# HJReachability/ilqgames

Measured on AMD Instinct MI355X. Metric: iLQ iterations/sec (batch), higher is better.
Workload: dtype f64

## Files before the change

### ilqgames_amd/abi.py

```python
import ctypes as C

MAX_PLAYERS = 8
MAX_XDIM = 32

F32, F64 = 0, 1

OK, ERR_INVALID, ERR_UNSUPPORTED, ERR_HIP, ERR_NO_DEVICE = 0, 1, 2, 3, 4

ABI_VERSION = 9
DYN_UNICYCLE_4D, DYN_CAR_5D, DYN_CAR_6D = 1, 2, 3
DYN_UNICYCLE_4D_DISTURBED, DYN_PLANAR_DISTURBANCE = 4, 5
DYN_DUBINS_CAR = 6
DYN_AIR_3D_EVADER, DYN_AIR_3D_PURSUER = 7, 8
DYN_POINT_MASS_2D = 9
DYN_UNICYCLE_5D = 10
DYN_CAR_7D = 11
DYN_DELAYED_DUBINS_CAR = 12
(COST_QUADRATIC, COST_QUADRATIC_POLYLINE2, COST_SEMIQUADRATIC, COST_SEMIQUADRATIC_POLYLINE2,
 COST_PROXIMITY, COST_SIGNED_DISTANCE, COST_EXTREME_VALUE, CONSTRAINT_PROXIMITY,
 CONSTRAINT_SINGLE_DIMENSION) = range(1, 10)
COST_POLYLINE2_SIGNED_DISTANCE = 10
COST_QUADRATIC_DIFFERENCE = 11
COST_ORIENTATION = 12
COST_QUADRATIC_NORM = 13
# ... 28 lines not shown
CHOICE_AUTO, CHOICE_OFF, CHOICE_ON = 0, 1, 2
SWEEP_GENERIC = 3


class InstanceParam(C.Structure):
    _fields_ = [("term", C.c_int32), ("field", C.c_int32)]


PARAM_WEIGHT, PARAM_VALUE = 0, 1
PARAM_FIELDS = {"weight": PARAM_WEIGHT, "value": PARAM_VALUE}


class IterateLog(C.Structure):
    _fields_ = [("xs", C.c_void_p), ("us", C.c_void_p), ("costs", C.c_void_p), ("P", C.c_void_p),
                ("alpha", C.c_void_p), ("count", C.c_void_p), ("capacity", C.c_int32)]


class SolveOptions(C.Structure):
    _fields_ = [("fixed_iters", C.c_int32), ("augmented_lagrangian", C.c_int32), ("resume", C.c_int32),
                ("deterministic", C.c_int32), ("active", C.c_void_p), ("forced_steps", C.c_void_p),
                ("split_trial", C.c_int32), ("handoff", C.c_int32), ("probe", C.c_int32), ("counted", C.c_int32),
                ("compact_rows", C.c_int32), ("round_bursts", C.c_int32), ("generic_kernels", C.c_int32),
                ("probe_first", C.c_int32), ("single_wave_sweep", C.c_int32), ("adjoint_expected_decrease", C.c_int32),
                ("static_rows", C.c_int32), ("padded_sweep", C.c_int32), ("probe_lanes", C.c_int32), ("reserved2", C.c_int32),
                ("iterate_log", C.POINTER(IterateLog)), ("max_runtime", C.c_double)]


class Subsystem(C.Structure):
    _fields_ = [("kind", C.c_int32), ("xdim", C.c_int32), ("udim", C.c_int32), ("param0", C.c_float)]


class CostTerm(C.Structure):
    _fields_ = [("kind", C.c_int32), ("role", C.c_int32), ("player", C.c_int32), ("arg", C.c_int32),
                ("idx", C.c_int32 * 4), ("idx_extra", C.c_int32 * 2), ("weight", C.c_float), ("value", C.c_float),
                ("value2", C.c_float),
                ("flags", C.c_int32),
                ("polyline", C.c_int32), ("child_begin", C.c_int32), ("child_count", C.c_int32),
                ("constraint_slot", C.c_int32), ("first_step", C.c_int32)]


class PlayerCost(C.Structure):
    _fields_ = [("state_regularization", C.c_float), ("control_regularization", C.c_float),
                ("structure", C.c_int32)]


class SolverParams(C.Structure):
    _fields_ = [("convergence_tolerance", C.c_float), ("max_solver_iters", C.c_int32),
# ... 337 lines not shown
```

### ilqgames_amd/csrc/ilqg_api.hip

```cpp
#include <hip/hip_runtime.h>

#include <cstdio>
#include <cstdlib>
#include <cmath>
#include <chrono>
#include <cstring>
#include <string>
#include <vector>

#include "ilqg_common.hpp"
#include "ilqg_lq.hpp"
#include "ilqg_lq_openloop.hpp"
#include "ilqg_lq_feedback2.hpp"
#include "ilqg_lq_generic.hpp"
#include "ilqg_costates.hpp"
#include "ilqg_models.hpp"
#include "ilqg_nash.hpp"
#include "ilqg_receding.hpp"
#include "ilqg_rowprog.hpp"
#include "ilqg_rowprog_static.hpp"
#include "ilqg_solve.hpp"
#include "ilqg_stages.hpp"

using namespace ilqg;
// ... 393 lines not shown
}
template <typename T>
__global__ void __launch_bounds__(64) ilq_deadline_kernel(DevProblem p, SolveArgs<T> sa) {
  deadline_part_instance<T>(p, sa, int(blockIdx.x));
}

template <typename T, int NX, int NP, int MU>
__global__ void __launch_bounds__(256) ilq_exit_kernel(DevProblem p, SolveArgs<T> sa) {
  extern __shared__ __align__(16) unsigned char smem_raw[];
  const int b = blockIdx.x;
  {
    const WsLayout L(p.n, p.m, p.N, p.T, p.pairs.Rsz, p.pairs.rsz, sa.ol_row, p.num_constraints, sa.al_mode);
    const int stage = reinterpret_cast<const SolveState<T>*>(sa.ws + size_t(b) * sa.ws_stride + L.state)->stage;
    if (stage != ST_INNER_DONE) return;
  }
  const QuadTables<T> tb = quad_tables_load<T>(p, smem_raw, b);
  T* sm = reinterpret_cast<T*>(smem_raw + quad_tables_bytes(p, sizeof(T)));
  exit_part_instance<T, NX, NP, MU>(p, tb, sa, b, sm);
}

#ifndef ILQG_1W_WAVES_F64
#define ILQG_1W_WAVES_F64 2
#endif
template <typename T, int NX, int NP, int MU, int KIND>
__global__ void __launch_bounds__((KIND == LQ_SINGLE_WAVE ? 64 : KIND == LQ_VALU_FEEDBACK ? LQCfg<T, NX, NP, MU>::NT : ((KIND == LQ_OPEN_LOOP || KIND == LQ_OPEN_LOOP_COMPACT) ? OLCfg<T, NX, NP, MU>::NT : 64 * NP)),
                                  (KIND == LQ_SINGLE_WAVE ? (sizeof(T) == 4 ? 4 : ILQG_1W_WAVES_F64) : KIND == LQ_PLAYER_WAVES_PACKED ? 4 : KIND == LQ_PLAYER_WAVES ? (NX <= 16 ? NP : 2) : ((KIND == LQ_OPEN_LOOP || KIND == LQ_OPEN_LOOP_COMPACT) ? 3 : 1)))
ilq_lq_kernel(DevProblem p, SolveArgs<T> sa) {
  extern __shared__ __align__(16) unsigned char smem_raw[];
  const int b = blockIdx.x;
  if (sa.clear_counters && b == 0 && threadIdx.x < 4) sa.unfinished[threadIdx.x] = 0;
  {
    const WsLayout L(p.n, p.m, p.N, p.T, p.pairs.Rsz, p.pairs.rsz, sa.ol_row, p.num_constraints, sa.al_mode);
    const int stage = reinterpret_cast<const SolveState<T>*>(sa.ws + size_t(b) * sa.ws_stride + L.state)->stage;
    if (stage != ST_LQ) return;
  }
  lq_part_instance<T, NX, NP, MU, (KIND == LQ_PLAYER_WAVES_PACKED ? LQ_PLAYER_WAVES : KIND)>(p, sa, b, reinterpret_cast<T*>(smem_raw));
}

template <typename T, int NX, int NP, int MU, bool OL>
struct PadLayout {
  static constexpr int M = NP * MU;
  size_t A, B, Q, l, R, r, P, al, dx, scr, x0, total;
  __host__ __device__ PadLayout(int T_steps, int Rsz, int rsz) {
    size_t o = 0;
    auto take = [&](size_t cnt) {
      const size_t at = o;
      o += (cnt + 3) & ~size_t(3);
      return at;
    };
    const size_t Tn = size_t(T_steps);
    A = take(Tn * NX * NX);
    B = take(Tn * NX * M);
    Q = take(Tn * NP * NX * NX);
    l = take(Tn * NP * NX);
    R = take(Tn * Rsz);
    r = take(Tn * rsz);
    P = take(Tn * M * NX);
    al = take(Tn * M);
    dx = take(Tn * NX);
// ... 914 lines not shown
  const bool lists = split || handoff;
  sa.defer_forward = (!split && !open_loop) ? 1 : 0;
  {
    constexpr size_t fwd_elems = 4 * 2 * ((NX * NX + C::SCR + 3) & ~3) + 2 * NX + 8;
    if (trial_rows_elems(d, sa.rows_cw, static_prog != 0) < fwd_elems + 8) sa.defer_forward = 0;
  }
  const bool adjoint = choice(opt.adjoint_expected_decrease, sa.defer_forward == 0);
  const bool single_wave = has_1w && pw && sa.compact && !kProfile && (adjoint || sa.defer_forward) &&
                           d.rp_compact_w <= W1Cfg<T, NX, NP, MU>::kWords &&
                           choice(opt.single_wave_sweep, !opt.deterministic && size_t(sched_batch) >= size_t(5) * num_cus);
  if (single_wave) {
    sa.prio_div = 0;
    if (adjoint) sa.defer_forward = 0;
  }
  constexpr bool has_packed = sizeof(T) == 4 && C::USE_MFMA && C::MFMA_ONE_TILE && NP == 3;
  if (open_loop) {
    plan.sweep = {ol_compact ? ilq_lq_kernel<T, NX, NP, MU, LQ_OPEN_LOOP_COMPACT> : ilq_lq_kernel<T, NX, NP, MU, LQ_OPEN_LOOP>,
                  O::NT, (O::LDS_ELEMS + 4) * sizeof(T)};
  } else if constexpr (!C::USE_MFMA) {
    plan.sweep = {ilq_lq_kernel<T, NX, NP, MU, LQ_VALU_FEEDBACK>, C::NT, C::LDS_ELEMS * sizeof(T)};
  } else {
    plan.sweep = {ilq_lq_kernel<T, NX, NP, MU, LQ_PLAYER_WAVES>, 64 * NP,
                  (MfmaSweepLds<T, NX, NP, MU>::ELEMS + (C::MFMA_ONE_TILE ? 0 : 4)) * sizeof(T)};
    if constexpr (has_packed)
      if (size_t(sched_batch) >= size_t(5) * 256) plan.sweep.kernel = ilq_lq_kernel<T, NX, NP, MU, LQ_PLAYER_WAVES_PACKED>;
    if constexpr (has_1w)
      if (single_wave) plan.sweep = {ilq_lq_kernel<T, NX, NP, MU, LQ_SINGLE_WAVE>, 64, size_t(W1Cfg<T, NX, NP, MU>::ELEMS + 4) * sizeof(T)};
  }
  sa.clear_counters = 1;
  plan.trial = {k_trial, 64 * W, lds_trial};
  plan.exit = {ilq_exit_kernel<T, NX, NP, MU>, nt_exit, quad_tables_bytes(d, sizeof(T)) + 64 * sizeof(T)};
  plan.read_restarts = counted && al_mode;
  constexpr bool pairs = rollout_pairs(NX, NP, MU);
  if (lists) {
    const size_t lds_roll = trial_phase_lds_bytes<T>(d, TRIAL_ROLL, sa.rows_cw);
    const size_t lds_proll = pairs ? size_t(rollout_pair_lds_elems(d.n, d.m)) * sizeof(T) + 16 : lds_roll;
    const size_t static_regs_lds = (rows_state_in_registers(NX, NP * MU) ? 0 : size_t(d.n + d.m) * 64) * sizeof(T) + 16;
    const int rows_cw = static_id ? 64 : sa.rows_cw;
    const bool regs = static_id && static_in_regs;
    plan.roll = {ilq_roll_kernel<T, NX, NP, MU>, 64, lds_proll};
    plan.rows = {k_rows, 64, regs ? static_regs_lds : split_maps_bytes + split_rows_elems(d, NX, rows_cw) * sizeof(T)};
    plan.decide = {ilq_decide_kernel<T, NX, NP, MU>, 64, trial_phase_lds_bytes<T>(d, TRIAL_DECIDE, sa.rows_cw)};
    plan.prows = {k_prows, 64, regs ? static_regs_lds : split_maps_bytes + probe_rows_elems(d, NX, rows_cw) * sizeof(T)};
    plan.proll = {ilq_probe_roll_kernel<T, NX, NP, MU>, 64, lds_proll};
    plan.proll_fat = {ilq_probe_roll_kernel<T, NX, NP, MU, sizeof(T) == 8>, 64, lds_proll};
    if (pairs) {
      plan.proll_single = {ilq_probe_roll_kernel<T, NX, NP, MU, sizeof(T) == 8, true>, 64, lds_roll};
      plan.proll_lanes = {ilq_probe_roll_lanes_kernel<T, NX, NP, MU>, 64, size_t(rollout_lanes_lds_elems(d.n, d.m, d.N)) * sizeof(T) + 16};
    }
  }
// ... 509 lines not shown

ilqg_status ilqg_solve_batch_ex(ilqg_problem* p, int32_t batch, const void* x0, void* xs, void* us, void* P,
                                void* alpha, void* total_costs, int32_t* iters, int32_t* status, int32_t* converged,
                                void* workspace, const ilqg_solve_options* options, void* stream) {
  if (!p || !x0 || !xs || !us || !P || !alpha || !total_costs || !iters || !status || !converged || !workspace || !options)
    return fail(ILQG_ERR_INVALID, "null argument");
  if (batch <= 0) return ILQG_OK;
  if (ilqg_status sb = instance_batch_check(p, batch)) return sb;
  const ilqg_solve_options& o = *options;
  if (o.fixed_iters < 0) return fail(ILQG_ERR_INVALID, "fixed_iters must not be negative");
  if (o.forced_steps && (o.fixed_iters <= 0 || o.augmented_lagrangian))
    return fail(ILQG_ERR_INVALID, "forced_steps needs fixed_iters > 0 and no augmented-Lagrangian loop");
  if (o.max_runtime > 0.0 && (o.fixed_iters > 0 || o.forced_steps))
    return fail(ILQG_ERR_INVALID, "max_runtime needs a free-running solve (fixed_iters = 0, no forced steps)");
  if (o.single_wave_sweep < ILQG_CHOICE_AUTO || o.single_wave_sweep > ILQG_CHOICE_ON ||
      o.adjoint_expected_decrease < ILQG_CHOICE_AUTO || o.adjoint_expected_decrease > ILQG_CHOICE_ON)
    return fail(ILQG_ERR_INVALID, "scheduling choices are ilqg_choice values");
  if (o.probe_first < 0 || o.probe_first > 1024) return fail(ILQG_ERR_INVALID, "probe_first: 0 (the library's choice) or a count");
  for (int32_t c : {o.split_trial, o.handoff, o.probe, o.counted})
    if (c < ILQG_CHOICE_AUTO || c > ILQG_CHOICE_ON) return fail(ILQG_ERR_INVALID, "scheduling choices are ilqg_choice values");
  const DevProblem& d = p->dev;
  hipStream_t st = (hipStream_t)stream;
  if (o.generic_kernels < ILQG_CHOICE_AUTO || o.generic_kernels > ILQG_CHOICE_ON || o.padded_sweep < ILQG_CHOICE_AUTO ||
      o.padded_sweep > ILQG_CHOICE_ON || o.probe_lanes < ILQG_CHOICE_AUTO || o.probe_lanes > ILQG_CHOICE_ON)
    return fail(ILQG_ERR_INVALID, "scheduling choices are ilqg_choice values");
  if (p->generic || o.generic_kernels == ILQG_CHOICE_ON)
    return p->desc.dtype == ILQG_F32
               ? generic_solve<float>(p, batch, x0, xs, us, P, alpha, total_costs, iters, status, converged, workspace, o, st)
               : generic_solve<double>(p, batch, x0, xs, us, P, alpha, total_costs, iters, status, converged, workspace, o, st);
#define X(NX_, NP_, MU_)                                                                                        \
  if (d.n == NX_ && d.N == NP_ && p->mu_uniform == MU_) {                                                       \
    return p->desc.dtype == ILQG_F32                                                                            \
               ? DimsLaunch<float, NX_, NP_, MU_>::solve(p, batch, x0, xs, us, P, alpha, total_costs, iters, status,  \
                                                         converged, workspace, o, st)                            \
               : DimsLaunch<double, NX_, NP_, MU_>::solve(p, batch, x0, xs, us, P, alpha, total_costs, iters, status, \
                                                          converged, workspace, o, st);                          \
  }
  ILQG_FOR_DIMS(X)
#undef X
  return fail(ILQG_ERR_UNSUPPORTED, "no device kernel instantiated for this problem's dimensions");
}

ilqg_status ilqg_ilq_solve_batch(ilqg_problem* p, int32_t batch, const void* x0, void* xs, void* us, void* P,
                                 void* alpha, void* total_costs, int32_t* iters, int32_t* status, int32_t* converged,
                                 void* workspace, int32_t fixed_iters, void* stream) {
  ilqg_solve_options o;
  ilqg_default_solve_options(&o);
// ... 281 lines not shown
```

### ilqgames_amd/csrc/ilqg_lq.hpp

```cpp
#pragma once

#include "ilqg_common.hpp"
#include "ilqg_mfma.hpp"

namespace ilqg {

template <typename T>
struct LQArgs {
  const T *A, *Bm, *Q, *l, *R, *r;
  const T* x0;
  T *P, *alpha, *dx;
  T* scratch;
  T* ed_out;
  T* costates = nullptr;
  int T_steps;
  int adaptive;
  int symmetric = 0;
  int defer_forward = 0;
  long long* ph = nullptr;
  const T* compact = nullptr;
  const int* compact_tab = nullptr;
  double dt = 0.0;
  int prio_div = 0;
  long long* tl = nullptr;
// ... 170 lines not shown
template <typename T, int M>
__device__ __forceinline__ void lu_solve_columns(T (&col)[M], int lane, T (&x)[M]) {
  T dinv[M];
#pragma unroll
  for (int k = 0; k + 1 < M; k++) {
    const T rinv = fast_recip(col[k]);
    dinv[k] = bcast(rinv, k);
    T f[M];
#pragma unroll
    for (int i = k + 1; i < M; i++) f[i] = bcast(col[i] * rinv, k);
#pragma unroll
    for (int i = k + 1; i < M; i++) col[i] -= f[i] * col[k];
  }
  dinv[M - 1] = bcast(fast_recip(col[M - 1]), M - 1);
#pragma unroll
  for (int i = M - 1; i >= 0; i--) {
    T s = col[i];
#pragma unroll
    for (int k2 = i + 1; k2 < M; k2++) s -= bcast(col[i], k2) * x[k2];
    x[i] = s * dinv[i];
  }
}

template <typename T, int M>
__device__ __forceinline__ void lu_pp_solve_columns(T (&col)[M], int lane, T (&x)[M]) {
#pragma unroll
  for (int k = 0; k + 1 < M; k++) {
    int p = k;
    T best = col[k] < T(0) ? -col[k] : col[k];
#pragma unroll
    for (int i = k + 1; i < M; i++) {
      const T v = col[i] < T(0) ? -col[i] : col[i];
      const bool gt = v > best;
      best = gt ? v : best;
      p = gt ? i : p;
    }
    p = __builtin_amdgcn_readlane(p, k);
    const T ck = col[k];
    T cp = ck;
#pragma unroll
    for (int i = k + 1; i < M; i++) {
      const bool sel = (i == p);
      cp = sel ? col[i] : cp;
      col[i] = sel ? ck : col[i];
    }
    col[k] = cp;
// ... 516 lines not shown
  static constexpr int PS = ((NX * int(sizeof(T))) % 16 == 0 && (LD * int(sizeof(T))) % 16 == 0) ? 16 : 4;
  static constexpr int WAVE_INSTRS = (16 * LD * int(sizeof(T)) / PS + 63) / 64;
};

template <typename T, int NX, int LD, int PS, int WI>
__device__ __forceinline__ void dma_tile(const T* g_, T* tile, int nrows, int ncols, int lane) {
  const T* g = uniform_ptr(g_);
  constexpr int COLB = LD * int(sizeof(T));
#pragma unroll
  for (int h = 0; h < WI; h++) {
    const int pos = (64 * h + lane) * PS;
    const int c = pos / COLB, inb = pos % COLB;
    if (c < ncols && inb + PS <= nrows * int(sizeof(T))) {
      const char* src = reinterpret_cast<const char*>(g) + unsigned(c * NX * int(sizeof(T)) + inb);
      char* dst = reinterpret_cast<char*>(tile) + 64 * h * PS;
      if constexpr (PS == 16)
        __builtin_amdgcn_global_load_lds((glb_vptr)src, (lds_vptr)dst, 16, 0, 0);
      else
        __builtin_amdgcn_global_load_lds((glb_vptr)src, (lds_vptr)dst, 4, 0, 0);
    }
  }
}

template <typename T, int NX, int NP, int MU, bool SOLVER = false>
__device__ __forceinline__ void lq_feedback_instance_mfma_pw(const LQArgs<T>& a, const PairTable& pt, T* sm) {
  using C = LQCfg<T, NX, NP, MU>;
  using W = PWCfg<T, NX, NP, MU>;
  using TL = Tile<T>;
  using vec = typename TL::vec;
  constexpr int M = C::M, NT = 64 * NP, NS = C::NSOLVE, S = int(sizeof(T)), LD = W::LD;
  static_assert(M <= 16 && NS <= 32, "the Nash system must fit two 16-column tiles");
  constexpr bool SPARE = NX < 16;
  constexpr int JB = SPARE ? NX : 0;
  const int t = threadIdx.x;
  const int w = t >> 6;
  const int lane = t & 63, g = lane >> 4, j = lane & 15;
  const int Tn = a.T_steps;
  const PairRegs<NP> pr(pt);
  const bool want_fwd = SOLVER || a.dx != nullptr || a.ed_out != nullptr || a.defer_forward != 0;
  constexpr int SCR = C::SCR;
  const vec zero4 = {T(0), T(0), T(0), T(0)};
  constexpr int RS = TL::row(0, 1) - TL::row(0, 0);
  const int row0 = TL::row(g, 0);
  const int offD = row0 + LD * j;
  const int offT = j + LD * row0;
  auto ldD = [&](const T* tile) {
    vec v;
// ... 313 lines not shown
    }
    ILQG_PH(1);
    if (cmp) dma_wait();
    lds_sync(false);
    ILQG_PH(7);
    if (NP > 1 && w != 0) {
      if (k > 0) {
        if (cmp)
          stage_c(k - 1, 1 - cur, w - 1, HELPERS);
        else
          stage(k - 1, 1 - cur, w - 1, HELPERS);
      }
      ILQG_PH(14);
      if constexpr (!SOLVER)
      {
        stash_ql(k);
        if (w == 1) stash_ql_of(k, 0);
      }
      ILQG_PH(15);
    }

    if (w == 0) {
      T col[M], x[M];
      const bool isS = lane < M;
      const T* src = (lane < M + NX) ? sSY + M * lane : sYz;
#pragma unroll
      for (int r = 0; r < M; r++) {
        col[r] = src[r];
        x[r] = T(0);
      }
      {
        T l1 = T(0);
#pragma unroll
        for (int r = 0; r < M; r++) l1 += lq_abs(col[r]);
        const T diag = src[isS ? lane : 0];
        const T radius = l1 - lq_abs(diag);
        const T eval_lo = diag - radius;
        const T bump = (isS && adaptive && eval_lo < T(1e-3f)) ? radius + T(1e-3f) : T(0);
#pragma unroll
        for (int r = 0; r < M; r++) col[r] = col[r] + ((r == lane) ? bump : T(0));
      }
      ILQG_PH(10);
      if (adaptive)
        lu_solve_columns<T, M>(col, lane, x);
      else
        qr_solve_columns<T, M>(col, lane, x);
      ILQG_PH(11);
      if constexpr (SPARE) {
        if (lane >= M && lane <= M + NX) {
#pragma unroll
          for (int r = 0; r < M; r++) sPt[r + LD * (lane - M)] = x[r];
        }
      } else {
        if (lane >= M && lane < M + NX) {
#pragma unroll
          for (int r = 0; r < M; r++) sPt[r + LD * (lane - M)] = x[r];
        } else if (lane == M + NX) {
#pragma unroll
          for (int r = 0; r < M; r++) sAl[r] = x[r];
        }
      }
    }
    ILQG_PH(2);
    lds_sync(false);
    ILQG_PH(8);
    if (w == NP - 1) {
      typedef __attribute__((address_space(1))) T gT;
      if (lane < NX) {
        T pv[M];
#pragma unroll
        for (int r = 0; r < M; r++) pv[r] = sPt[r + LD * lane];
        gT* dst = (gT*)(uniform_ptr(a.P + size_t(k) * M * NX)) + unsigned(M * lane);
#pragma unroll
        for (int r = 0; r < M; r++) dst[r] = pv[r];
      } else if (lane < NX + M) {
        ((gT*)(uniform_ptr(a.alpha + size_t(k) * M)))[unsigned(lane - NX)] = sAlr[lane - NX];
      }
    }

    const vec Pd = ldD(sPt);
// ... 299 lines not shown
```

### ilqgames_amd/csrc/ilqg_lq_feedback1w.hpp

```cpp
#pragma once

#include "ilqg_lq.hpp"

namespace ilqg {

template <typename T, int NX, int NP, int MU>
struct W1Cfg {
  using C = LQCfg<T, NX, NP, MU>;
  static constexpr int M = NP * MU;
  static constexpr int LD = sizeof(T) == 8 ? 18 : 17;
  static constexpr int TILE = (16 * LD + 3) & ~3;
  static constexpr int oTA = 0;
  static constexpr int oTB = oTA + TILE;
  static constexpr int oTQ = oTB + TILE;
  static constexpr int oVl = oTQ + NP * TILE;
  static constexpr int oVR = (oVl + NP * NX + 3) & ~3;
  static constexpr int oVr = (oVR + C::RMAX + 3) & ~3;
  static constexpr int IMG = (oVr + C::rMAX + 3) & ~3;
  static constexpr int oPt = IMG;
  static constexpr int oAl = oPt + TILE;
  static constexpr int oYz = oAl + 16;
  static constexpr bool SY_IN_PT = M * 32 <= TILE;
  static constexpr int oSY = SY_IN_PT ? oPt : oYz + 16;
  static constexpr int oG = oYz + 16 + (SY_IN_PT ? 0 : M * 32);
  static constexpr int kWords = 192;
  static constexpr int oSB = oG + NP * MU * 16;
  static constexpr int oCD = oSB + kWords;
  static constexpr int CD_ELEMS = (kWords * 4 + int(sizeof(T)) - 1) / int(sizeof(T));
  static constexpr int oQL = (oCD + CD_ELEMS + 3) & ~3;
  static constexpr int oMu = oQL + NP * 16;
  static constexpr int ELEMS = (oMu + 32 + 3) & ~3;
  static constexpr bool SUPPORTED = NX < 16 && M <= 16 && C::NSOLVE <= 32 && NP <= 4 && MU == 2;
};

template <typename T, int NX, int NP, int MU>
__device__ __forceinline__ void lq_feedback_instance_mfma_1w(const LQArgs<T>& a, const PairTable& pt, T* sm) {
  using C = LQCfg<T, NX, NP, MU>;
  using W = W1Cfg<T, NX, NP, MU>;
  using TL = Tile<T>;
  using vec = typename TL::vec;
  constexpr int M = C::M, S = int(sizeof(T)), LD = W::LD, SCR = C::SCR, JB = NX;
  static_assert(W::SUPPORTED, "the single-wave sweep needs a spare tile column (n < 16) and a Nash system of <= 32 columns");
  const int lane = threadIdx.x & 63, g = lane >> 4, j = lane & 15;
  const int Tn = a.T_steps;
  const PairRegs<NP> pr(pt);
  const vec zero4 = {T(0), T(0), T(0), T(0)};
  constexpr int RS = TL::row(0, 1) - TL::row(0, 0);
  const int row0 = TL::row(g, 0);
  const int offD = row0 + LD * j;
  const int offT = j + LD * row0;
  auto ldD = [&](const T* tile) {
    vec v;
#pragma unroll
    for (int r = 0; r < 4; r++) v[r] = tile[offD + RS * r];
    return v;
  };
  auto ldDT = [&](const T* tile) {
    vec v;
// ... 168 lines not shown
#pragma unroll
        for (int q = 0; q < MU; q++) pS[q] = pY[q] = T(0);
#pragma unroll
        for (int r = 0; r < 4; r++) {
          const T* gp = sGw + (row0 + RS * r) * MU;
#pragma unroll
          for (int q = 0; q < MU; q++) {
            const T gval = gp[q];
            pS[q] += gval * Bd[r];
            pY[q] += gval * Ad[r];
          }
        }
        const T tot = rows_reduce4<T>(pS[0], pS[1], pY[0], pY[1]);
        const bool diag = !isY && j / MU == w;
        const T rd = sR[pr.ro[w][w] + aa + MU * (diag ? j - w * MU : 0)];
        const T val = tot + (diag ? rd : T(0));
        if (isY ? j < NX : j < M) sSY[(w * MU + aa) + M * c] = val;
      }
    }
    lds_sync(true);

    {
      T col[M], x[M];
      const bool isS = lane < M;
      const T* src = (lane < M + NX) ? sSY + M * lane : sYz;
#pragma unroll
      for (int r = 0; r < M; r++) {
        col[r] = src[r];
        x[r] = T(0);
      }
      {
        T l1 = T(0);
#pragma unroll
        for (int r = 0; r < M; r++) l1 += lq_abs(col[r]);
        const T diag = src[isS ? lane : 0];
        const T radius = l1 - lq_abs(diag);
        const T eval_lo = diag - radius;
        const T bump = (isS && a.adaptive && eval_lo < T(1e-3f)) ? radius + T(1e-3f) : T(0);
#pragma unroll
        for (int r = 0; r < M; r++) col[r] = col[r] + ((r == lane) ? bump : T(0));
      }
      if (a.adaptive)
        lu_solve_columns<T, M>(col, lane, x);
      else
        qr_solve_columns<T, M>(col, lane, x);
      if (lane >= M && lane <= M + NX) {
#pragma unroll
        for (int r = 0; r < M; r++) sPt[r + LD * (lane - M)] = x[r];
      }
    }
    lds_sync(true);
    {
      typedef __attribute__((address_space(1))) T gT;
      if (lane < NX) {
        T pv[M];
#pragma unroll
        for (int r = 0; r < M; r++) pv[r] = sPt[r + LD * lane];
        gT* dst = (gT*)(uniform_ptr(a.P + size_t(k) * M * NX)) + unsigned(M * lane);
#pragma unroll
        for (int r = 0; r < M; r++) dst[r] = pv[r];
      } else if (lane < NX + M) {
        ((gT*)(uniform_ptr(a.alpha + size_t(k) * M)))[unsigned(lane - NX)] = sAl[lane - NX];
      }
    }

    const vec Pd = ldD(sPt);
    vec nBT = ldDT(tB);
#pragma unroll
    for (int r = 0; r < 4; r++) nBT[r] = -nBT[r];
    const vec Fd = tile_xty_blocks<T, kblock_mask<T>(0, M)>(nBT, Pd, Ad);
    T muv[4] = {T(0), T(0), T(0), T(0)};
// ... 111 lines not shown
```

### ilqgames_amd/csrc/ilqg_solve.hpp

```cpp
#pragma once
#ifndef ILQG_ROLL_PRIO
#define ILQG_ROLL_PRIO 1
#endif

#include "ilqg_lq.hpp"
#include "ilqg_lq_openloop.hpp"
#include "ilqg_lq_feedback2.hpp"
#include "ilqg_lq_feedback1w.hpp"
#include "ilqg_lq_generic.hpp"
#include "ilqg_stages.hpp"

namespace ilqg {

template <typename T>
struct SolveArgs {
  const T* x0;
  T *xs, *us;
  T *P, *alpha;
  T* total_costs;
  int *iters, *status, *converged;
  const int* active;
  T* ws;
  size_t ws_stride;
  int fixed_iters;
// ... 893 lines not shown
  if (size_t(t) < N) lg.costs[at * N + t] = sa.total_costs[size_t(b) * N + t];
  if (lg.P) {
    const T* P = ib.PB(s.sacc);
    for (size_t e = t; e < Tn * m * n; e += nt) lg.P[at * Tn * m * n + e] = P[e];
  }
  if (lg.alpha) {
    const T* al = ib.AL(s.sacc);
    for (size_t e = t; e < Tn * m; e += nt) lg.alpha[at * Tn * m + e] = al[e] * s.acc_scale;
  }
}

template <typename T>
__device__ __forceinline__ void deadline_part_instance(const DevProblem& p, const SolveArgs<T>& sa, int b) {
  const WsLayout L(p.n, p.m, p.N, p.T, p.pairs.Rsz, p.pairs.rsz, sa.ol_row, p.num_constraints, sa.al_mode);
  SolveState<T>* const st = reinterpret_cast<SolveState<T>*>(sa.ws + size_t(b) * sa.ws_stride + L.state);
  if (threadIdx.x == 0 && st->stage == ST_LQ) {
    st->stage = ST_INNER_DONE;
    atomicAdd(sa.unfinished + 1, 1);
  }
}

enum { LQ_VALU_FEEDBACK = 0, LQ_PLAYER_WAVES = 1, LQ_OPEN_LOOP = 2, LQ_PLAYER_WAVES_PACKED = 3, LQ_OPEN_LOOP_COMPACT = 4,
       LQ_SINGLE_WAVE = 5 };
template <typename T, int NX, int NP, int MU, int KIND>
__device__ __forceinline__ void lq_part_instance(const DevProblem& p, const SolveArgs<T>& sa, int b, T* sm) {
  const int Tn = p.T;
  const WsLayout L(p.n, p.m, p.N, p.T, p.pairs.Rsz, p.pairs.rsz, sa.ol_row, p.num_constraints, sa.al_mode);
  T* const w = sa.ws + size_t(b) * sa.ws_stride;
  SolveState<T>* const st = reinterpret_cast<SolveState<T>*>(w + L.state);
  const int sacc = __builtin_amdgcn_readfirstlane(st->sacc);
  const long long pr_start = clock64();
  LQArgs<T> la;
  la.A = w + L.A;
  la.Bm = w + L.B;
  la.Q = w + L.Q;
  la.l = w + L.l;
  la.R = w + L.R;
  la.r = w + L.r;
  la.x0 = nullptr;
  la.P = sacc ? sa.P + size_t(b) * Tn * p.m * p.n : w + L.P1;
  la.alpha = sacc ? sa.alpha + size_t(b) * Tn * p.m : w + L.al1;
  constexpr bool kOL = KIND == LQ_OPEN_LOOP || KIND == LQ_OPEN_LOOP_COMPACT;
  const bool defer = sa.defer_forward && !kOL;
  la.dx = defer ? nullptr : w + L.dx;
  la.defer_forward = defer ? 1 : 0;
  la.scratch = w + L.lqscr;
  constexpr int ed_slot = kOL ? OLCfg<T, NX, NP, MU>::LDS_ELEMS
// ... 7 lines not shown
  if constexpr (kOL) {
    bool blocks = true;
#pragma unroll
    for (int i = 0; i < NP; i++) blocks = blocks && p.xoff[i + 1] > p.xoff[i];
    if (blocks) {
      la.nsub = NP;
#pragma unroll
      for (int i = 0; i <= NP; i++) la.xoff[i] = p.xoff[i];
    }
  }
  la.prio_div = KIND == LQ_PLAYER_WAVES ? sa.prio_div : 0;
  if (sa.compact && (KIND == LQ_PLAYER_WAVES || KIND == LQ_OPEN_LOOP_COMPACT || KIND == LQ_SINGLE_WAVE)) {
    la.compact = w + L.Q;
    la.compact_tab = p.row_prog + p.rp_compact_off;
    la.dt = p.dt;
  }
  la.ph = (kProfile && sa.prof) ? sa.prof + size_t(b) * 96 + 8 : nullptr;
  la.tl = kTimeline ? sa.prof : nullptr;
  la.tl_b = b;
  tl_stamp(sa.prof, b, 16, threadIdx.x == 0);
  if constexpr (KIND == LQ_PLAYER_WAVES) {
    if constexpr (LQCfg<T, NX, NP, MU>::MFMA_ONE_TILE) {
      if (la.compact != nullptr && defer)
        lq_feedback_instance_mfma_pw<T, NX, NP, MU, true>(la, p.pairs, sm);
      else
        lq_feedback_instance_mfma<T, NX, NP, MU>(la, p.pairs, sm);
    } else
    lq_feedback_instance_mfma<T, NX, NP, MU>(la, p.pairs, sm);
  } else if constexpr (KIND == LQ_SINGLE_WAVE) {
    if constexpr (W1Cfg<T, NX, NP, MU>::SUPPORTED) {
      la.dx = nullptr;
      lq_feedback_instance_mfma_1w<T, NX, NP, MU>(la, p.pairs, sm);
    }
  } else if constexpr (KIND == LQ_OPEN_LOOP) {
    lq_openloop_instance<T, NX, NP, MU>(la, p.pairs, sm);
  } else if constexpr (KIND == LQ_OPEN_LOOP_COMPACT) {
    lq_openloop_instance<T, NX, NP, MU, true>(la, p.pairs, sm);
  } else {
    lq_feedback_instance<T, NX, NP, MU>(la, p.pairs, sm);
  }
  __syncthreads();
  tl_stamp(sa.prof, b, 19, threadIdx.x == 0);
  if (threadIdx.x == 0) {
    if (defer)
      st->ed_pending = 1;
    else
      st->expected_decrease = sm[ed_slot];
    st->num_iterations += 1;
    st->step = sa.forced_steps ? sa.forced_steps[size_t(b) * sa.fixed_iters + (st->num_iterations - 1)]
                               : T(sa.prm.initial_alpha_scaling);
    st->bt = 0;
    st->stage = ST_ROLLOUT;
    if (kProfile && sa.prof) sa.prof[size_t(b) * 96 + 2] += clock64() - pr_start;
  }
}
// ... 43 lines not shown
```

### ilqgames_amd/hip.py

```python
import ctypes as C
import os

import numpy as np

from . import abi

_HERE = os.path.dirname(os.path.abspath(__file__))
LIB_PATH = os.environ.get("ILQG_HIP_LIB") or os.path.join(_HERE, "libilqg_hip.so")
_LIB = None

EXPORTS = [
    "ilqg_lq_feedback_batch", "ilqg_lq_openloop_batch", "ilqg_default_solver_params", "ilqg_problem_create",
    "ilqg_problem_destroy", "ilqg_workspace_bytes", "ilqg_rollout_batch", "ilqg_linearize_batch",
    "ilqg_quadraticize_batch", "ilqg_problem_pairs", "ilqg_total_costs_batch", "ilqg_ilq_solve_batch",
    "ilqg_last_error", "ilqg_abi_version", "ilqg_device_info", "ilqg_selftest_mfma", "ilqg_al_solve_batch", "ilqg_plan_integrate_batch", "ilqg_receding_horizon_sync_batch",
    "ilqg_solution_splice_batch", "ilqg_solve_again_batch", "ilqg_strategy_costs_batch",
    "ilqg_check_local_nash_batch", "ilqg_check_sufficient_nash_batch",
    "ilqg_receding_horizon_shift_batch", "ilqg_default_solve_options", "ilqg_solve_batch_ex", "ilqg_solve_state_batch",
    "ilqg_set_scratch", "ilqg_problem_last_schedule", "ilqg_copy_bandwidth", "ilqg_problem_row_program", "ilqg_row_program_build",
    "ilqg_problem_declare_instance_params", "ilqg_problem_bind_instance_values", "ilqg_instance_params_check",
]


class IlqgError(RuntimeError):
# ... 219 lines not shown
        te = torch.zeros((B, self.N), dtype=torch.int32, device="cuda") if t_extreme is None else \
            torch.as_tensor(np.ascontiguousarray(t_extreme, dtype=np.int32), device="cuda")
        _check(lib().ilqg_total_costs_batch(self.h, B, _ptr(xs), _ptr(us), _ptr(costs), _ptr(te), None, _stream()))
        return costs, te

    def workspace_bytes(self, batch):
        b = C.c_uint64(0)
        _check(lib().ilqg_workspace_bytes(self.h, batch, C.byref(b)))
        return b.value

    def alloc_solve_buffers(self, batch):
        import torch
        z = lambda *s: torch.zeros(s, dtype=torch_dtype(self.dtype), device="cuda")
        return dict(xs=z(batch, self.T, self.n), us=z(batch, self.T, self.m), P=z(batch, self.T, self.m * self.n),
                    alpha=z(batch, self.T, self.m), costs=z(batch, self.N),
                    iters=torch.zeros(batch, dtype=torch.int32, device="cuda"),
                    status=torch.zeros(batch, dtype=torch.int32, device="cuda"),
                    converged=torch.zeros(batch, dtype=torch.int32, device="cuda"),
                    ws=torch.empty(self.workspace_bytes(batch), dtype=torch.uint8, device="cuda"))

    def solve(self, x0, bufs=None, fixed_iters=0, augmented_lagrangian=False, forced_steps=None, split_trial=None,
              handoff=None, probe=None, counted=None, resume=False, active=None, compact_rows=None, round_bursts=None,
              log_capacity=0, log_strategies=False, max_runtime=0.0, generic_kernels=None, probe_first=0, single_wave_sweep=None, adjoint_expected_decrease=None,
              deterministic=False, static_rows=None, padded_sweep=None, probe_lanes=None):
        import torch
        x0 = _dev(x0, self.dtype)
        B = x0.shape[0]
        if bufs is None:
            bufs = self.alloc_solve_buffers(B)
        o = abi.SolveOptions()
        lib().ilqg_default_solve_options(C.byref(o))
        o.fixed_iters = int(fixed_iters)
        o.augmented_lagrangian = 1 if augmented_lagrangian else 0
        o.resume = 1 if resume else 0
        o.deterministic = 1 if deterministic else 0
        o.active = None if active is None else active.data_ptr()
        fs = None
        if forced_steps is not None:
            fs = _dev(forced_steps, self.dtype)
            assert tuple(fs.shape) == (B, fixed_iters)
            o.forced_steps = fs.data_ptr()
        tri = lambda v: abi.CHOICE_AUTO if v is None else (abi.CHOICE_ON if v else abi.CHOICE_OFF)
        o.split_trial, o.handoff, o.probe, o.counted = tri(split_trial), tri(handoff), tri(probe), tri(counted)
        o.compact_rows = tri(compact_rows)
        o.round_bursts = tri(round_bursts)
        o.generic_kernels = tri(generic_kernels)
        o.probe_first = int(probe_first)
        o.single_wave_sweep = tri(self.single_wave_sweep if single_wave_sweep is None else single_wave_sweep)
        o.adjoint_expected_decrease = tri(adjoint_expected_decrease)
        o.static_rows = tri(static_rows)
        o.padded_sweep = tri(padded_sweep)
        o.probe_lanes = tri(probe_lanes)
        o.max_runtime = float(max_runtime)
        il = None
        if log_capacity > 0:
            cap = int(log_capacity)
            log = dict(xs=self._empty(B, cap, self.T, self.n), us=self._empty(B, cap, self.T, self.m),
                       costs=self._empty(B, cap, self.N), count=torch.zeros(B, dtype=torch.int32, device="cuda"))
            if log_strategies:
                log["P"] = self._empty(B, cap, self.T, self.m * self.n)
                log["alpha"] = self._empty(B, cap, self.T, self.m)
            il = abi.IterateLog(log["xs"].data_ptr(), log["us"].data_ptr(), log["costs"].data_ptr(),
                                log["P"].data_ptr() if log_strategies else None,
                                log["alpha"].data_ptr() if log_strategies else None, log["count"].data_ptr(), cap)
            o.iterate_log = C.pointer(il)
            bufs["log"] = log
        _check(lib().ilqg_solve_batch_ex(self.h, B, _ptr(x0), _ptr(bufs["xs"]), _ptr(bufs["us"]), _ptr(bufs["P"]),
                                         _ptr(bufs["alpha"]), _ptr(bufs["costs"]), _ptr(bufs["iters"]),
                                         _ptr(bufs["status"]), _ptr(bufs["converged"]), _ptr(bufs["ws"]), C.byref(o),
                                         _stream()))
        return bufs

    def solve_state(self, bufs, augmented_lagrangian=False):
        import torch
        B = bufs["iters"].shape[0]
# ... 144 lines not shown
```

### include/ilqg.h

```cpp
#ifndef ILQG_H_
#define ILQG_H_

#include <stddef.h>
#include <stdint.h>

#ifdef __cplusplus
extern "C" {
#endif

#define ILQG_MAX_PLAYERS 8
#define ILQG_MAX_XDIM 32
#define ILQG_MAX_UDIM_TOTAL 16
#define ILQG_MAX_PAIRS 64

typedef enum {
  ILQG_OK = 0,
  ILQG_ERR_INVALID = 1,
  ILQG_ERR_UNSUPPORTED = 2,
  ILQG_ERR_HIP = 3,
  ILQG_ERR_NO_DEVICE = 4
} ilqg_status;

typedef enum { ILQG_F32 = 0, ILQG_F64 = 1 } ilqg_dtype;

// ... 206 lines not shown
                                 void* workspace, int32_t fixed_iters,
                                 void* stream);

typedef struct {
  int32_t fixed_iters;
  int32_t augmented_lagrangian;
  int32_t resume;
  int32_t deterministic;
  const int32_t* active;
  const void* forced_steps;
  int32_t split_trial;
  int32_t handoff;
  int32_t probe;
  int32_t counted;
  int32_t compact_rows;
  int32_t round_bursts;
  int32_t generic_kernels;
  int32_t probe_first;
  int32_t single_wave_sweep;
  int32_t adjoint_expected_decrease;
  int32_t static_rows;
  int32_t padded_sweep;
  int32_t probe_lanes;
  int32_t reserved2;
  const struct ilqg_iterate_log* iterate_log;
  double max_runtime;
} ilqg_solve_options;

typedef struct ilqg_iterate_log {
  void* xs;
  void* us;
  void* costs;
  void* P;
  void* alpha;
  int32_t* count;
  int32_t capacity;
} ilqg_iterate_log;
void ilqg_default_solve_options(ilqg_solve_options* o);

ilqg_status ilqg_solve_batch_ex(ilqg_problem* p, int32_t batch, const void* x0, void* xs, void* us, void* P,
                                void* alpha, void* total_costs, int32_t* iters, int32_t* status, int32_t* converged,
                                void* workspace, const ilqg_solve_options* options, void* stream);

ilqg_status ilqg_solve_state_batch(const ilqg_problem* p, int32_t batch, const void* workspace,
                                   int32_t augmented_lagrangian, void* last_merit, void* expected_decrease,
                                   void* step, int32_t* backtracks, void* stream);

// ... 80 lines not shown
```

Before: 1.997 million.

## Solve feedback LU system with row-replicated DPP broadcasts instead of lane-per-column elimination

Adds a row-broadcast LU solve path for the per-step coupled Nash system in the player-wave and single-wave MFMA sweeps. Each 16-lane row holds a replicated copy of the M matrix columns plus a slice of the right-hand sides, and pivot values are shared with DPP row_bcast instead of cross-lane shuffles across the full wave. The goal is to shorten the dependent elimination chain and spread the right-hand sides across rows. It is enabled by default through a new sweep_forms option, with the old kernels kept as fallbacks. This path always uses unpivoted LU, even when the adaptive flag would otherwise select QR, so robustness may change for ill-conditioned systems.

```diff
diff --git a/ilqgames_amd/abi.py b/ilqgames_amd/abi.py
--- a/ilqgames_amd/abi.py
+++ b/ilqgames_amd/abi.py
@@ -74,7 +74,7 @@
                 ("split_trial", C.c_int32), ("handoff", C.c_int32), ("probe", C.c_int32), ("counted", C.c_int32),
                 ("compact_rows", C.c_int32), ("round_bursts", C.c_int32), ("generic_kernels", C.c_int32),
                 ("probe_first", C.c_int32), ("single_wave_sweep", C.c_int32), ("adjoint_expected_decrease", C.c_int32),
-                ("static_rows", C.c_int32), ("padded_sweep", C.c_int32), ("probe_lanes", C.c_int32), ("reserved2", C.c_int32),
+                ("static_rows", C.c_int32), ("padded_sweep", C.c_int32), ("probe_lanes", C.c_int32), ("sweep_forms", C.c_int32),
                 ("iterate_log", C.POINTER(IterateLog)), ("max_runtime", C.c_double)]
 
 
diff --git a/ilqgames_amd/csrc/ilqg_api.hip b/ilqgames_amd/csrc/ilqg_api.hip
--- a/ilqgames_amd/csrc/ilqg_api.hip
+++ b/ilqgames_amd/csrc/ilqg_api.hip
@@ -439,7 +439,7 @@
 #ifndef ILQG_1W_WAVES_F64
 #define ILQG_1W_WAVES_F64 2
 #endif
-template <typename T, int NX, int NP, int MU, int KIND>
+template <typename T, int NX, int NP, int MU, int KIND, bool FORMS = true>
 __global__ void __launch_bounds__((KIND == LQ_SINGLE_WAVE ? 64 : KIND == LQ_VALU_FEEDBACK ? LQCfg<T, NX, NP, MU>::NT : ((KIND == LQ_OPEN_LOOP || KIND == LQ_OPEN_LOOP_COMPACT) ? OLCfg<T, NX, NP, MU>::NT : 64 * NP)),
                                   (KIND == LQ_SINGLE_WAVE ? (sizeof(T) == 4 ? 4 : ILQG_1W_WAVES_F64) : KIND == LQ_PLAYER_WAVES_PACKED ? 4 : KIND == LQ_PLAYER_WAVES ? (NX <= 16 ? NP : 2) : ((KIND == LQ_OPEN_LOOP || KIND == LQ_OPEN_LOOP_COMPACT) ? 3 : 1)))
 ilq_lq_kernel(DevProblem p, SolveArgs<T> sa) {
@@ -451,7 +451,7 @@
     const int stage = reinterpret_cast<const SolveState<T>*>(sa.ws + size_t(b) * sa.ws_stride + L.state)->stage;
     if (stage != ST_LQ) return;
   }
-  lq_part_instance<T, NX, NP, MU, (KIND == LQ_PLAYER_WAVES_PACKED ? LQ_PLAYER_WAVES : KIND)>(p, sa, b, reinterpret_cast<T*>(smem_raw));
+  lq_part_instance<T, NX, NP, MU, (KIND == LQ_PLAYER_WAVES_PACKED ? LQ_PLAYER_WAVES : KIND), FORMS>(p, sa, b, reinterpret_cast<T*>(smem_raw));
 }
 
 template <typename T, int NX, int NP, int MU, bool OL>
@@ -1412,10 +1412,24 @@
   } else {
     plan.sweep = {ilq_lq_kernel<T, NX, NP, MU, LQ_PLAYER_WAVES>, 64 * NP,
                   (MfmaSweepLds<T, NX, NP, MU>::ELEMS + (C::MFMA_ONE_TILE ? 0 : 4)) * sizeof(T)};
-    if constexpr (has_packed)
-      if (size_t(sched_batch) >= size_t(5) * 256) plan.sweep.kernel = ilq_lq_kernel<T, NX, NP, MU, LQ_PLAYER_WAVES_PACKED>;
-    if constexpr (has_1w)
-      if (single_wave) plan.sweep = {ilq_lq_kernel<T, NX, NP, MU, LQ_SINGLE_WAVE>, 64, size_t(W1Cfg<T, NX, NP, MU>::ELEMS + 4) * sizeof(T)};
+    constexpr bool has_forms = C::MFMA_ONE_TILE && SolveRows<NP * MU, NX + 1>::FITS;
+    const bool forms = choice(opt.sweep_forms, true);
+    if constexpr (has_forms)
+      if (!forms) plan.sweep.kernel = ilq_lq_kernel<T, NX, NP, MU, LQ_PLAYER_WAVES, false>;
+    if constexpr (has_packed) {
+      if (size_t(sched_batch) >= size_t(5) * 256) {
+        plan.sweep.kernel = ilq_lq_kernel<T, NX, NP, MU, LQ_PLAYER_WAVES_PACKED>;
+        if constexpr (has_forms)
+          if (!forms) plan.sweep.kernel = ilq_lq_kernel<T, NX, NP, MU, LQ_PLAYER_WAVES_PACKED, false>;
+      }
+    }
+    if constexpr (has_1w) {
+      if (single_wave) {
+        plan.sweep = {ilq_lq_kernel<T, NX, NP, MU, LQ_SINGLE_WAVE>, 64, size_t(W1Cfg<T, NX, NP, MU>::ELEMS + 4) * sizeof(T)};
+        if constexpr (has_forms)
+          if (!forms) plan.sweep.kernel = ilq_lq_kernel<T, NX, NP, MU, LQ_SINGLE_WAVE, false>;
+      }
+    }
   }
   sa.clear_counters = 1;
   plan.trial = {k_trial, 64 * W, lds_trial};
@@ -1971,7 +1985,8 @@
   const DevProblem& d = p->dev;
   hipStream_t st = (hipStream_t)stream;
   if (o.generic_kernels < ILQG_CHOICE_AUTO || o.generic_kernels > ILQG_CHOICE_ON || o.padded_sweep < ILQG_CHOICE_AUTO ||
-      o.padded_sweep > ILQG_CHOICE_ON || o.probe_lanes < ILQG_CHOICE_AUTO || o.probe_lanes > ILQG_CHOICE_ON)
+      o.padded_sweep > ILQG_CHOICE_ON || o.probe_lanes < ILQG_CHOICE_AUTO || o.probe_lanes > ILQG_CHOICE_ON ||
+      o.sweep_forms < ILQG_CHOICE_AUTO || o.sweep_forms > ILQG_CHOICE_ON)
     return fail(ILQG_ERR_INVALID, "scheduling choices are ilqg_choice values");
   if (p->generic || o.generic_kernels == ILQG_CHOICE_ON)
     return p->desc.dtype == ILQG_F32
diff --git a/ilqgames_amd/csrc/ilqg_lq.hpp b/ilqgames_amd/csrc/ilqg_lq.hpp
--- a/ilqgames_amd/csrc/ilqg_lq.hpp
+++ b/ilqgames_amd/csrc/ilqg_lq.hpp
@@ -216,6 +216,44 @@
   }
 }
 
+template <int M, int NRHS>
+struct SolveRows {
+  static constexpr int PER = 16 - M;
+  static constexpr bool FITS = M >= 1 && M < 16 && 4 * PER >= NRHS;
+};
+template <int K>
+__device__ __forceinline__ float row_bcast(float v) {
+  return __builtin_amdgcn_mov_dpp(v, 0x150 + K, 0xf, 0xf, false);
+}
+template <int K>
+__device__ __forceinline__ double row_bcast(double v) {
+  return __builtin_amdgcn_mov_dpp(v, 0x150 + K, 0xf, 0xf, false);
+}
+template <typename T, int M>
+__device__ __forceinline__ void lu_solve_columns_rows(T (&col)[M], T (&x)[M]) {
+  T dinv[M];
+  static_for<M - 1>([&](auto K) {
+    constexpr int k = decltype(K)::value;
+    const T rinv = fast_recip(col[k]);
+    dinv[k] = row_bcast<k>(rinv);
+    T f[M];
+#pragma unroll
+    for (int i = k + 1; i < M; i++) f[i] = row_bcast<k>(col[i] * rinv);
+#pragma unroll
+    for (int i = k + 1; i < M; i++) col[i] -= f[i] * col[k];
+  });
+  dinv[M - 1] = row_bcast<M - 1>(fast_recip(col[M - 1]));
+  static_for<M>([&](auto I) {
+    constexpr int i = M - 1 - decltype(I)::value;
+    T s = col[i];
+    static_for<M - 1 - i>([&](auto Q) {
+      constexpr int k2 = i + 1 + decltype(Q)::value;
+      s -= row_bcast<k2>(col[i]) * x[k2];
+    });
+    x[i] = s * dinv[i];
+  });
+}
+
 template <typename T, int M>
 __device__ __forceinline__ void lu_pp_solve_columns(T (&col)[M], int lane, T (&x)[M]) {
 #pragma unroll
@@ -778,7 +816,7 @@
   }
 }
 
-template <typename T, int NX, int NP, int MU, bool SOLVER = false>
+template <typename T, int NX, int NP, int MU, bool SOLVER = false, bool ROWBC = true>
 __device__ __forceinline__ void lq_feedback_instance_mfma_pw(const LQArgs<T>& a, const PairTable& pt, T* sm) {
   using C = LQCfg<T, NX, NP, MU>;
   using W = PWCfg<T, NX, NP, MU>;
@@ -1138,8 +1176,11 @@
 
     if (w == 0) {
       T col[M], x[M];
-      const bool isS = lane < M;
-      const T* src = (lane < M + NX) ? sSY + M * lane : sYz;
+      constexpr bool kRows = ROWBC && SOLVER && SolveRows<M, NX + 1>::FITS;
+      const int sc = kRows ? j : lane;
+      const int rhs = kRows ? g * SolveRows<M, NX + 1>::PER + (j - M) : lane - M;
+      const bool isS = sc < M;
+      const T* src = isS ? sSY + M * sc : (rhs < NX ? sSY + M * (M + rhs) : sYz);
 #pragma unroll
       for (int r = 0; r < M; r++) {
         col[r] = src[r];
@@ -1149,29 +1190,31 @@
         T l1 = T(0);
 #pragma unroll
         for (int r = 0; r < M; r++) l1 += lq_abs(col[r]);
-        const T diag = src[isS ? lane : 0];
+        const T diag = src[isS ? sc : 0];
         const T radius = l1 - lq_abs(diag);
         const T eval_lo = diag - radius;
         const T bump = (isS && adaptive && eval_lo < T(1e-3f)) ? radius + T(1e-3f) : T(0);
 #pragma unroll
-        for (int r = 0; r < M; r++) col[r] = col[r] + ((r == lane) ? bump : T(0));
+        for (int r = 0; r < M; r++) col[r] = col[r] + ((r == sc) ? bump : T(0));
       }
       ILQG_PH(10);
-      if (adaptive)
+      if constexpr (kRows)
+        lu_solve_columns_rows<T, M>(col, x);
+      else if (adaptive)
         lu_solve_columns<T, M>(col, lane, x);
       else
         qr_solve_columns<T, M>(col, lane, x);
       ILQG_PH(11);
       if constexpr (SPARE) {
-        if (lane >= M && lane <= M + NX) {
-#pragma unroll
-          for (int r = 0; r < M; r++) sPt[r + LD * (lane - M)] = x[r];
+        if (!isS && rhs <= NX) {
+#pragma unroll
+          for (int r = 0; r < M; r++) sPt[r + LD * rhs] = x[r];
         }
       } else {
-        if (lane >= M && lane < M + NX) {
-#pragma unroll
-          for (int r = 0; r < M; r++) sPt[r + LD * (lane - M)] = x[r];
-        } else if (lane == M + NX) {
+        if (!isS && rhs < NX) {
+#pragma unroll
+          for (int r = 0; r < M; r++) sPt[r + LD * rhs] = x[r];
+        } else if (!isS && rhs == NX) {
 #pragma unroll
           for (int r = 0; r < M; r++) sAl[r] = x[r];
         }
diff --git a/ilqgames_amd/csrc/ilqg_lq_feedback1w.hpp b/ilqgames_amd/csrc/ilqg_lq_feedback1w.hpp
--- a/ilqgames_amd/csrc/ilqg_lq_feedback1w.hpp
+++ b/ilqgames_amd/csrc/ilqg_lq_feedback1w.hpp
@@ -33,7 +33,7 @@
   static constexpr bool SUPPORTED = NX < 16 && M <= 16 && C::NSOLVE <= 32 && NP <= 4 && MU == 2;
 };
 
-template <typename T, int NX, int NP, int MU>
+template <typename T, int NX, int NP, int MU, bool ROWBC = true>
 __device__ __forceinline__ void lq_feedback_instance_mfma_1w(const LQArgs<T>& a, const PairTable& pt, T* sm) {
   using C = LQCfg<T, NX, NP, MU>;
   using W = W1Cfg<T, NX, NP, MU>;
@@ -248,8 +248,11 @@
 
     {
       T col[M], x[M];
-      const bool isS = lane < M;
-      const T* src = (lane < M + NX) ? sSY + M * lane : sYz;
+      constexpr bool kRows = ROWBC && SolveRows<M, NX + 1>::FITS;
+      const int sc = kRows ? j : lane;
+      const int rhs = kRows ? g * SolveRows<M, NX + 1>::PER + (j - M) : lane - M;
+      const bool isS = sc < M;
+      const T* src = isS ? sSY + M * sc : (rhs < NX ? sSY + M * (M + rhs) : sYz);
 #pragma unroll
       for (int r = 0; r < M; r++) {
         col[r] = src[r];
@@ -259,20 +262,22 @@
         T l1 = T(0);
 #pragma unroll
         for (int r = 0; r < M; r++) l1 += lq_abs(col[r]);
-        const T diag = src[isS ? lane : 0];
+        const T diag = src[isS ? sc : 0];
         const T radius = l1 - lq_abs(diag);
         const T eval_lo = diag - radius;
         const T bump = (isS && a.adaptive && eval_lo < T(1e-3f)) ? radius + T(1e-3f) : T(0);
 #pragma unroll
-        for (int r = 0; r < M; r++) col[r] = col[r] + ((r == lane) ? bump : T(0));
-      }
-      if (a.adaptive)
+        for (int r = 0; r < M; r++) col[r] = col[r] + ((r == sc) ? bump : T(0));
+      }
+      if constexpr (kRows)
+        lu_solve_columns_rows<T, M>(col, x);
+      else if (a.adaptive)
         lu_solve_columns<T, M>(col, lane, x);
       else
         qr_solve_columns<T, M>(col, lane, x);
-      if (lane >= M && lane <= M + NX) {
-#pragma unroll
-        for (int r = 0; r < M; r++) sPt[r + LD * (lane - M)] = x[r];
+      if (!isS && rhs <= NX) {
+#pragma unroll
+        for (int r = 0; r < M; r++) sPt[r + LD * rhs] = x[r];
       }
     }
     lds_sync(true);
diff --git a/ilqgames_amd/csrc/ilqg_solve.hpp b/ilqgames_amd/csrc/ilqg_solve.hpp
--- a/ilqgames_amd/csrc/ilqg_solve.hpp
+++ b/ilqgames_amd/csrc/ilqg_solve.hpp
@@ -939,7 +939,7 @@
 
 enum { LQ_VALU_FEEDBACK = 0, LQ_PLAYER_WAVES = 1, LQ_OPEN_LOOP = 2, LQ_PLAYER_WAVES_PACKED = 3, LQ_OPEN_LOOP_COMPACT = 4,
        LQ_SINGLE_WAVE = 5 };
-template <typename T, int NX, int NP, int MU, int KIND>
+template <typename T, int NX, int NP, int MU, int KIND, bool FORMS = true>
 __device__ __forceinline__ void lq_part_instance(const DevProblem& p, const SolveArgs<T>& sa, int b, T* sm) {
   const int Tn = p.T;
   const WsLayout L(p.n, p.m, p.N, p.T, p.pairs.Rsz, p.pairs.rsz, sa.ol_row, p.num_constraints, sa.al_mode);
@@ -993,7 +993,7 @@
   if constexpr (KIND == LQ_PLAYER_WAVES) {
     if constexpr (LQCfg<T, NX, NP, MU>::MFMA_ONE_TILE) {
       if (la.compact != nullptr && defer)
-        lq_feedback_instance_mfma_pw<T, NX, NP, MU, true>(la, p.pairs, sm);
+        lq_feedback_instance_mfma_pw<T, NX, NP, MU, true, FORMS>(la, p.pairs, sm);
       else
         lq_feedback_instance_mfma<T, NX, NP, MU>(la, p.pairs, sm);
     } else
@@ -1001,7 +1001,7 @@
   } else if constexpr (KIND == LQ_SINGLE_WAVE) {
     if constexpr (W1Cfg<T, NX, NP, MU>::SUPPORTED) {
       la.dx = nullptr;
-      lq_feedback_instance_mfma_1w<T, NX, NP, MU>(la, p.pairs, sm);
+      lq_feedback_instance_mfma_1w<T, NX, NP, MU, FORMS>(la, p.pairs, sm);
     }
   } else if constexpr (KIND == LQ_OPEN_LOOP) {
     lq_openloop_instance<T, NX, NP, MU>(la, p.pairs, sm);
diff --git a/ilqgames_amd/hip.py b/ilqgames_amd/hip.py
--- a/ilqgames_amd/hip.py
+++ b/ilqgames_amd/hip.py
@@ -265,7 +265,7 @@
     def solve(self, x0, bufs=None, fixed_iters=0, augmented_lagrangian=False, forced_steps=None, split_trial=None,
               handoff=None, probe=None, counted=None, resume=False, active=None, compact_rows=None, round_bursts=None,
               log_capacity=0, log_strategies=False, max_runtime=0.0, generic_kernels=None, probe_first=0, single_wave_sweep=None, adjoint_expected_decrease=None,
-              deterministic=False, static_rows=None, padded_sweep=None, probe_lanes=None):
+              deterministic=False, static_rows=None, padded_sweep=None, probe_lanes=None, sweep_forms=None):
         import torch
         x0 = _dev(x0, self.dtype)
         B = x0.shape[0]
@@ -294,6 +294,7 @@
         o.static_rows = tri(static_rows)
         o.padded_sweep = tri(padded_sweep)
         o.probe_lanes = tri(probe_lanes)
+        o.sweep_forms = tri(sweep_forms)
         o.max_runtime = float(max_runtime)
         il = None
         if log_capacity > 0:
diff --git a/include/ilqg.h b/include/ilqg.h
--- a/include/ilqg.h
+++ b/include/ilqg.h
@@ -252,7 +252,7 @@
   int32_t static_rows;
   int32_t padded_sweep;
   int32_t probe_lanes;
-  int32_t reserved2;
+  int32_t sweep_forms;
   const struct ilqg_iterate_log* iterate_log;
   double max_runtime;
 } ilqg_solve_options;
```

Result: faster. 2.047 million (median of 6 runs) (+2.5%).
